# mhw32/multimodal-vae-public

Measured on AMD Instinct MI355X. Metric: images/sec (MVAE train step), higher is better.
Workload: dtype f32; 1 GPU; mnist MVAE train step, n-latents 64, batch 512 per GPU; global_batch=512, parallelism=dp1, launch=hipGraph replay

## Files before the change

### include/mvae_hip.h

```cpp
#ifndef MVAE_HIP_H
#define MVAE_HIP_H

#include <stddef.h>
#include <stdint.h>

#ifdef __cplusplus
extern "C" {
#endif

#define MVAE_OK          0
#define MVAE_ERR_ARG    (-1)
#define MVAE_ERR_LAUNCH (-2)
#define MVAE_ERR_WS     (-3)
#define MVAE_ERR_COMM   (-4)

#define MVAE_ACT_SWISH   1
#define MVAE_ACCUMULATE  2

#define MVAE_POE_VARIANT_A 0
#define MVAE_POE_VARIANT_B 1
#define MVAE_POE_NO_PRIOR  4
#define MVAE_MAX_EXPERTS  32

typedef void *mvae_stream_t;
// ... 137 lines not shown
#define MVAE_LROUTE_G2S_32x32_K4     7
#define MVAE_LROUTE_IGS_64x32_K4     8
#define MVAE_LROUTE_IGS_64x32_K2     9
#define MVAE_LROUTE_IGS_32x64_K4    10
#define MVAE_LROUTE_IGS_32x64_K2    11
#define MVAE_LROUTE_IGS_32x32_K8    12
#define MVAE_LROUTE_IGS_32x32_K4    13
#define MVAE_LROUTE_IG_32x128       14
#define MVAE_LROUTE_IG_128x128      15
#define MVAE_LROUTE_IG_128x64       16
#define MVAE_LROUTE_IG_64x128       17
#define MVAE_LROUTE_IG_64x64_K4     18
#define MVAE_LROUTE_IG_64x64_K2     19
#define MVAE_LROUTE_IG_64x64        20
#define MVAE_LROUTE_IG_32x128_S     30
#define MVAE_LROUTE_IG_128x128_S    31
#define MVAE_LROUTE_IG_128x64_S     32
#define MVAE_LROUTE_IG_64x128_S     33
#define MVAE_LROUTE_IG_64x64_K4_S   34
#define MVAE_LROUTE_IG_64x64_K2_S   35
#define MVAE_LROUTE_IG_64x64_S      36
#define MVAE_LROUTE_DGRAD_SMALLN    40
#define MVAE_LROUTE_WGRAD_DIRECT_4  41
#define MVAE_LROUTE_WGRAD_DIRECT_8  42
#define MVAE_LROUTE_WGRAD_DIRECT_16 43
#define MVAE_LROUTE_WGRAD_BATCHED2      50
#define MVAE_LROUTE_WGRAD_BATCHED       51
#define MVAE_LROUTE_WGRAD_BATCHED_ADAM  52
int mvae_linear_route(int op, int G, int M, int N, int K, int ld_a, int ld_b, size_t gs_a, size_t gs_b, int aligned,
                      int fwd_form, int want_db, size_t ws_bytes, int *splits ,
                      int *finish );
int mvae_linear_wgrad_batched_route(const mvae_wgrad_item *items, int n_items, int adam, int *tile_rows ,
                                    int *tile_cols , int *waves );

int mvae_conv2d_gen_fwd(const float *x, const float *w, float *pre, float *act,
                        int B, int Cin, int H, int W, int Cout, int ks, int stride, int pad,
                        mvae_stream_t stream);
int mvae_conv2d_gen_dgrad(const float *dy, const float *w, float *dx, const float *pre_in,
                          int B, int Cin, int H, int W, int Cout, int ks, int stride, int pad,
                          void *ws, size_t ws_bytes, mvae_stream_t stream);
int mvae_conv2d_gen_wgrad(const float *dy, const float *x, float *dw,
                          int B, int Cin, int H, int W, int Cout, int ks, int stride, int pad,
                          int flags, void *ws, size_t ws_bytes, mvae_stream_t stream);
int mvae_convT2d_gen_fwd(const float *x, const float *w, float *pre, float *act,
                         int B, int Cin, int H, int W, int Cout, int ks, int stride, int pad,
                         void *ws, size_t ws_bytes, mvae_stream_t stream);
int mvae_convT2d_gen_dgrad(const float *dy, const float *w, float *dx, const float *pre_in,
                           int B, int Cin, int H, int W, int Cout, int ks, int stride, int pad,
                           mvae_stream_t stream);
int mvae_convT2d_gen_wgrad(const float *dy, const float *x, float *dw,
                           int B, int Cin, int H, int W, int Cout, int ks, int stride, int pad,
                           int flags, void *ws, size_t ws_bytes, mvae_stream_t stream);
size_t mvae_conv_gen_ws_bytes(int op, int B, int Cin, int H, int W, int Cout, int ks, int stride, int pad);
int mvae_conv_gen_supported(int transposed, int B, int Cin, int H, int W, int Cout, int ks, int stride, int pad);

size_t mvae_bn_ws_bytes(int G, int C, int n_per_group);
int mvae_bn_train_fwd(const float *x, const float *gamma, const float *beta, float *y,
                      float *save_mean, float *save_invstd,
                      float *running_mean, float *running_var,
                      int G, int B, int C, int HW, float eps, float momentum,
                      int n_updates, const int *n_updates_dev ,
                      int flags, void *ws, size_t ws_bytes, mvae_stream_t stream);
int mvae_bn_train_bwd(const float *dy, const float *x, const float *gamma, const float *beta,
                      const float *save_mean, const float *save_invstd,
                      float *dx, float *dgamma, float *dbeta,
                      int G, int B, int C, int HW, int flags,
// ... 325 lines not shown
```

### multimodal-vae-public_amd/_lib.py

```python
import ctypes
import os
from ctypes import c_double, c_float, c_int, c_size_t, c_uint64, c_void_p

_HERE = os.path.dirname(os.path.abspath(__file__))
LIB_PATH = os.path.join(_HERE, 'libmvae_hip.so')

MVAE_OK = 0
ERRORS = {-1: 'MVAE_ERR_ARG (bad shape / null pointer / unsupported stride)',
          -2: 'MVAE_ERR_LAUNCH (hip kernel launch failed)',
          -3: 'MVAE_ERR_WS (workspace too small)',
          -4: 'MVAE_ERR_COMM (RCCL not loadable, or an RCCL / HIP runtime call of mvae_comm_* failed)'}
COMM_ID_BYTES = 128
ACT_SWISH = 1
ACCUMULATE = 2
POE_NO_PRIOR = 4
POE_VARIANT = {'A': 0, 'B': 1, 'A-noprior': 0 | POE_NO_PRIOR, 'B-noprior': 1 | POE_NO_PRIOR}
MAX_EXPERTS = 32
STATS_TILE_ELEMS = 512
MAX_TERMS = 40
CONV_OPS = {'conv_fwd': 0, 'conv_dgrad': 1, 'conv_wgrad': 2, 'convT_fwd': 3, 'convT_fwd_stats': 4, 'convT_dgrad': 5,
            'convT_wgrad': 6}
CONV_ROUTES = {1: 'igemm', 2: 'igemm_pair', 3: 'gemm2', 4: 'conv_patch', 5: 'small_fwd16', 6: 'small_fwd32',
               7: 'dgrad_small3d', 8: 'dgrad_small3', 9: 'dgrad_small2', 10: 'dgrad_small', 11: 's1', 12: 's1_wide',
               13: 'patch8', 14: 'patch7', 15: 'patch16', 16: 'patch_stats', 17: 'wgrad_smallcin',
# ... 105 lines not shown
                                                 c_int, P]),
    'mvae_embedding_swish_bwd_grouped': (c_int, [P, c_int, c_size_t, P, c_size_t, P, c_size_t, P, c_int, c_int,
                                                 c_int, c_int, c_int, P]),
    'mvae_resample_ksize': (c_int, [c_int, c_int]),
    'mvae_resample_coeffs': (c_int, [c_int, c_int, P, P]),
    'mvae_resize_crop_u8_to_f32': (c_int, [P, P] + [c_int] * 8 + [P, P, c_int, P, P, c_int, c_int, c_int, P]),
    'mvae_u8_to_f32': (c_int, [P, P, c_size_t, P]),
    'mvae_poe_fwd': (c_int, [ctypes.POINTER(Experts), c_int, c_int, P, c_int, P, P, P, P, P,
                             c_int, c_int, c_int, P]),
    'mvae_poe_fwd_draw': (c_int, [ctypes.POINTER(Experts), c_int, c_int, P, c_int, P, c_uint64, P, c_uint64, P, P, P, P,
                                  c_int, c_int, c_int, P]),
    'mvae_poe_bwd': (c_int, [ctypes.POINTER(Experts), c_int, c_int, P, c_int, P, P, P, P, P, P, P, c_int,
                             ctypes.POINTER(ExpertGrads), c_int, c_int, c_int, c_int, P]),
    'mvae_poe_bwd_split': (c_int, [ctypes.POINTER(Experts), c_int, c_int, P, c_int, P, P, P, P,
                                   ctypes.POINTER(c_int), P, ctypes.POINTER(c_int), P, c_int,
                                   ctypes.POINTER(ExpertGrads), c_int, c_int, c_int, c_int, P]),
    'mvae_kl_rows_fwd': (c_int, [P, P, P, c_int, c_int, P]),
    'mvae_kl_rows_bwd': (c_int, [P, P, P, P, P, c_int, c_int, P]),
    'mvae_bce_rowsum_fwd': (c_int, [P, P, P, P, P, P] + [c_int] * 7 + [P]),
    'mvae_bce_rowsum_bwd': (c_int, [P, P, P, P, P] + [c_int] * 7 + [P]),
    'mvae_bce_route': (c_int, [c_int] * 4 + [ctypes.POINTER(c_int), ctypes.POINTER(c_int)]),
    'mvae_ce_fwd': (c_int, [P, P, P, P, P, c_int, c_int, c_int, c_int, P]),
    'mvae_ce_bwd': (c_int, [P, P, P, P, c_int, c_int, c_int, c_int, P]),
    'mvae_group_sums': (c_int, [P, P, P, P, c_int, c_int, c_int, P]),
    'mvae_conv_k4_repack_floats': (c_size_t, [c_int, P, c_int, c_int, c_int, c_int, c_int, c_int, c_int]),
    'mvae_conv_k4_repack_batched': (c_int, [ctypes.POINTER(RepackItem), c_int, P]),
    'mvae_convT2d_k4_stats_tiles': (c_size_t, [c_int] * 7),
    'mvae_convT2d_k4_fwd_stats': (c_int, [P, P, P, c_size_t] + [c_int] * 7 + [P, c_size_t, P]),
    'mvae_conv_k4_route': (c_int, [c_int] * 8 + [c_size_t, ctypes.POINTER(c_int)]),
    'mvae_linear_route': (c_int, [c_int] * 7 + [c_size_t, c_size_t, c_int, c_int, c_int, c_size_t, ctypes.POINTER(c_int),
                                  ctypes.POINTER(c_int)]),
    'mvae_linear_wgrad_batched_route': (c_int, [ctypes.POINTER(WgradItem), c_int, c_int, ctypes.POINTER(c_int),
                                                ctypes.POINTER(c_int), ctypes.POINTER(c_int)]),
    'mvae_conv2d_gen_fwd': (c_int, [P, P, P, P] + [c_int] * 8 + [P]),
    'mvae_conv2d_gen_dgrad': (c_int, [P, P, P, P] + [c_int] * 8 + [P, c_size_t, P]),
    'mvae_conv2d_gen_wgrad': (c_int, [P, P, P] + [c_int] * 9 + [P, c_size_t, P]),
    'mvae_convT2d_gen_fwd': (c_int, [P, P, P, P] + [c_int] * 8 + [P, c_size_t, P]),
    'mvae_convT2d_gen_dgrad': (c_int, [P, P, P, P] + [c_int] * 8 + [P]),
    'mvae_convT2d_gen_wgrad': (c_int, [P, P, P] + [c_int] * 9 + [P, c_size_t, P]),
    'mvae_conv_gen_ws_bytes': (c_size_t, [c_int] * 9),
    'mvae_conv_gen_supported': (c_int, [c_int] * 9),
    'mvae_bn_stats_merge': (c_int, [P, c_int, c_int, c_int, c_int, P, P, P, P, c_float, c_float, c_int, P, P]),
    'mvae_linear_wgrad_batched': (c_int, [ctypes.POINTER(WgradItem), c_int, P]),
    'mvae_linear_wgrad_batched_adam': (c_int, [ctypes.POINTER(WgradItem), c_int, ctypes.POINTER(AdamFuse), P]),
    'mvae_adam_prepare': (c_int, [P, ctypes.c_int64, c_double, c_double, c_double, P, P]),
    'mvae_elbo_reduce': (c_int, [ctypes.POINTER(ElboPart), c_int, P, c_int, P, c_size_t, P, c_uint64, P]),
    'mvae_elbo_reduce_prepare': (c_int, [ctypes.POINTER(ElboPart), c_int, P, c_int, P, c_size_t, P, c_uint64, P,
                                         ctypes.c_int64, c_double, c_double, c_double, P, P]),
    'mvae_philox_fill': (c_int, [P, c_size_t, c_int, c_float, c_uint64, P, c_uint64, P]),
    'mvae_randn': (c_int, [P, c_size_t, c_uint64, P, P]),
    'mvae_bernoulli': (c_int, [P, c_size_t, c_float, c_uint64, P, P]),
    'mvae_adam_step': (c_int, [P, P, P, P, c_size_t, c_double, c_double, c_double, c_double, c_float, P, P]),
    'mvae_adam_apply': (c_int, [P, P, P, P, c_size_t, c_double, c_double, c_double, c_double, c_float, P, P]),
    'mvae_adam_apply_at': (c_int, [P, P, P, P, c_size_t, c_double, c_double, c_double, c_double, c_float, P,
                                   ctypes.c_int64, P]),
    'mvae_adam_apply_coef': (c_int, [P, P, P, P, c_size_t, P, c_double, c_double, c_double, c_float, P]),
    'mvae_counter_add': (c_int, [P, ctypes.c_int64, P]),
    'mvae_trace_marker': (c_int, [c_int, P]),
    'mvae_fill': (c_int, [P, c_size_t, c_float, P]),
    'mvae_ingest': (c_int, [P, P, c_size_t, P, P, c_size_t, P, P, c_size_t, P]),
    'mvae_reparam_fwd': (c_int, [P, P, P, P, c_size_t, P]),
    'mvae_reparam_bwd': (c_int, [P, P, P, P, P, c_size_t, P]),
    'mvae_dropout_fanout_fwd': (c_int, [P, P, P, c_float, c_int, c_int, c_int, P]),
    'mvae_dropout_fanin_bwd': (c_int, [P, P, P, c_float, c_int, c_int, c_int, P]),
    'mvae_block_gather': (c_int, [P, P, P, c_int, c_size_t, P]),
    'mvae_block_scatter_add': (c_int, [P, P, P, c_int, c_int, c_size_t, P]),
# ... 94 lines not shown
```

### multimodal-vae-public_amd/csrc/linear.hip

```cpp
#include "gemm_core.h"
#include "gemm2.h"
#include "linear_direct.h"



MVAE_EXPORT int mvae_abi_version(void) { return 6; }

#ifdef MVAE_TUNING
MvaeTune g_mvae_tune = {0, 0, 0, 0, 0, 0, 0, 0};
MVAE_EXPORT void mvae_debug_set_tiling(int wm, int wn, int splits) {
    g_mvae_tune.wm = wm; g_mvae_tune.wn = wn; g_mvae_tune.splits = splits;
}
MVAE_EXPORT void mvae_debug_set_kwaves(int kw) { g_mvae_tune.kw = kw; }
MVAE_EXPORT void mvae_debug_set_small(int off, int waves) { g_mvae_tune.small_off = off; g_mvae_tune.small_waves = waves; }
MVAE_EXPORT void mvae_debug_set_split_target(long blocks) { g_mvae_tune.split_target = blocks; }
MVAE_EXPORT void mvae_debug_set_knockout(int mode) { g_mvae_tune.knockout = mode; }
#endif

MVAE_EXPORT size_t mvae_gemm_ws_bytes(int rows_out, int cols_out, int reduce_len) {
    if (rows_out <= 0 || cols_out <= 0 || reduce_len <= 0) return 0;
    size_t n = split_ws_floats(rows_out, cols_out, reduce_len);
    const size_t repack = (size_t)rows_out * cols_out;
    if (MVAE_TUNE(splits) > 0) n = (size_t)MVAE_TUNE(splits) * ((size_t)rows_out * cols_out + rows_out);
    const size_t smallcin = (size_t)512 * rows_out * cols_out;
// ... 417 lines not shown
        }
        case MVAE_LOP_BCE_FWD: case MVAE_LOP_CE_FWD:
            if (G != 1 || ld_a < K || ld_b < N || (op == MVAE_LOP_CE_FWD && N > 32)) return MVAE_ERR_ARG;
            r = linear_loss_route(a, ld_a, a, M, N, K);
            break;
        case MVAE_LOP_DGRAD:
            if (ld_a < N || ld_b < K) return MVAE_ERR_ARG;
            r = linear_dgrad_route(a, ld_a, a, M, N, K, ws, ws_bytes, gr);
            break;
        case MVAE_LOP_WGRAD:
            if (ld_a < N || ld_b < K) return MVAE_ERR_ARG;
            r = linear_wgrad_route(a, ld_a, a, ld_b, want_db != 0, M, N, K, ws, ws_bytes, gr);
            break;
        default: return MVAE_ERR_ARG;
    }
    if (r.route > 0) {
        if (splits) *splits = r.splits;
        if (finish) *finish = r.finish;
    }
    return r.route;
}

MVAE_EXPORT int mvae_linear_wgrad_batched_route(const mvae_wgrad_item *items, int n_items, int adam, int *tile_rows,
                                                int *tile_cols, int *waves) {
    WgradBatchArgs a;
    const int rc = wgrad_batch_table(items, n_items, adam != 0, a);
    if (rc != MVAE_OK) return rc;
    const WgradBatchRoute r = wgrad_batched_route(a, adam != 0);
    if (tile_rows) *tile_rows = r.tile_m;
    if (tile_cols) *tile_cols = r.tile_n;
    if (waves) *waves = r.waves;
    return r.route;
}
```

### multimodal-vae-public_amd/csrc/linear_direct.h

```cpp
#pragma once
#include "gemm_core.h"

namespace {

#ifdef MVAE_TUNING
#define MVAE_KO1 1
#define MVAE_KO2 2
#else
#define MVAE_KO1 0
#define MVAE_KO2 0
#endif
constexpr int WD_PD = 4;

struct AdamFuse {
    const float *grad_base; float *param, *m, *v; const float *coef;
    float b1, b2, omb1, omb2, eps, gscale;
    __device__ AdamCoef load() const {
        AdamCoef c;
        c.b1 = b1; c.b2 = b2; c.omb1 = omb1; c.omb2 = omb2; c.eps = eps; c.gscale = gscale;
        c.step_size = coef[0]; c.inv_sqrt_bc2 = coef[1];
        return c;
    }
    __device__ void update(const float *gptr, float g, const AdamCoef &c) const {
        const size_t off = (size_t)(gptr - grad_base);
        adam_one(param[off], m[off], v[off], g, c);
    }
};

template <bool ROWSUM, int KW, int MODE = 0, bool ADAM = false>
__device__ __forceinline__ void wgrad_direct_tile(const float *dy, int lddy, const float *x, int ldx,
                                                  const EpRowMajor &e, int I, int J, int M, float *db,
                                                  int db_accumulate, int tile_i, int tile_j,
                                                  const AdamFuse *af = nullptr) {
    extern __shared__ __attribute__((aligned(16))) float wd_lds[];
// ... 157 lines not shown
        for (int el = threadIdx.x; el < ADAM_ONLY_TILE; el += 64 * KW) {
            const int idx = local * ADAM_ONLY_TILE + el;
            if (idx < w.J) af->update(w.dw + idx, w.dw[idx], ac);
        }
        return;
    }
    const int tile_i = local / w.tiles_j, tile_j = local - tile_i * w.tiles_j;
    EpRowMajor e;
    e.out = w.dw; e.act = nullptr; e.ld = w.J; e.bias = nullptr; e.dpre = nullptr; e.ldp = 0;
    e.mask = nullptr; e.ldm = 0; e.mask_scale = 1.f; e.I = w.I; e.J = w.J; e.accumulate = w.accumulate;
    if (w.db) wgrad_direct_tile<true, KW, 0, ADAM>(w.dy, w.lddy, w.x, w.ldx, e, w.I, w.J, w.M, w.db, w.accumulate, tile_i, tile_j, af);
    else wgrad_direct_tile<false, KW, 0, ADAM>(w.dy, w.lddy, w.x, w.ldx, e, w.I, w.J, w.M, nullptr, 0, tile_i, tile_j, af);
}

#ifndef MVAE_WB2_PD22
#define MVAE_WB2_PD22 1
#endif
#ifndef MVAE_WB2_PD11
#define MVAE_WB2_PD11 2
#endif

constexpr int WB2_SEGS = 8;
struct WgradBatch2Args { WgradBatchItem it[WGRAD_BATCH_MAX]; int n; int seg[WB2_SEGS + 1]; };

__device__ __forceinline__ i32x4_t wb2_rsrc(BufBase b, unsigned off, unsigned extent) {
    const unsigned long long a = (((unsigned long long)b.hi << 32) | b.lo) + off;
    i32x4_t r;
    r.x = (int)(unsigned)a; r.y = (int)((unsigned)(a >> 32) & 0xffffu);
    const int left = (int)extent - (int)off;
    r.z = left > 0 ? left : 0; r.w = 0x00020000;
    return r;
}

template <int KW, int FM, int FN, int PD>
__device__ __forceinline__ void wgrad_tile2(const WgradBatchItem &w, int tile_i, int tile_j) {
    extern __shared__ __attribute__((aligned(16))) float wd_lds[];
    constexpr int TM = 32 * FM, TN = 32 * FN;
    const int t = threadIdx.x, lane = t & 63;
    const int kg = __builtin_amdgcn_readfirstlane(t >> 6);
    const int lcol = lane & 31, lrow = lane >> 5;
    const int i0 = tile_i * TM, j0 = tile_j * TN;
    const BufBase ba = buf_base(w.dy), bb = buf_base(w.x);
    const int M = __builtin_amdgcn_readfirstlane(w.M), I = __builtin_amdgcn_readfirstlane(w.I), J = __builtin_amdgcn_readfirstlane(w.J);
    const unsigned ulda = (unsigned)__builtin_amdgcn_readfirstlane(w.lddy) * 4u;
    const unsigned uldb = (unsigned)__builtin_amdgcn_readfirstlane(w.ldx) * 4u;
    const unsigned ext_a = (unsigned)(M - 1) * ulda + (unsigned)I * 4u;
    const unsigned ext_b = (unsigned)(M - 1) * uldb + (unsigned)J * 4u;
    int va[4], vb[4];
#pragma unroll
    for (int q = 0; q < 4; ++q) {
        va[q] = (int)((unsigned)(4 * lrow + q) * ulda + (unsigned)(i0 + lcol) * 4u);
        vb[q] = (int)((unsigned)(4 * lrow + q) * uldb + (unsigned)(j0 + lcol) * 4u);
    }
    const bool rs_block = w.db != nullptr && tile_j == 0;
    f32x16 acc[FM][FN];
#pragma unroll
    for (int a = 0; a < FM; ++a)
#pragma unroll
        for (int b = 0; b < FN; ++b)
#pragma unroll
            for (int r = 0; r < 16; ++r) acc[a][b][r] = 0.f;
    float rs[FM];
#pragma unroll
    for (int a = 0; a < FM; ++a) rs[a] = 0.f;

    const int nchunks = (M + 7) >> 3;
    const int n_it = (nchunks + KW - 1) / KW;
    float a0[PD][FM][4], b0[PD][FN][4], a1[PD][FM][4], b1[PD][FN][4];
    auto load_set = [&](int first, float (&as)[PD][FM][4], float (&bs)[PD][FN][4]) {
#pragma unroll
        for (int p = 0; p < PD; ++p) {
            const unsigned c = (unsigned)(kg + (first + p) * KW);
            const i32x4_t ra = wb2_rsrc(ba, c * 8u * ulda, ext_a), rb = wb2_rsrc(bb, c * 8u * uldb, ext_b);
#pragma unroll
            for (int q = 0; q < 4; ++q) {
#pragma unroll
                for (int f = 0; f < FM; ++f) as[p][f][q] = buf_load1(ra, va[q] + 128 * f);
#pragma unroll
                for (int f = 0; f < FN; ++f) bs[p][f][q] = buf_load1(rb, vb[q] + 128 * f);
            }
        }
    };
    auto use_set = [&](auto with_rs, const float (&as)[PD][FM][4], const float (&bs)[PD][FN][4]) {
#pragma unroll
        for (int p = 0; p < PD; ++p) {
#pragma unroll
            for (int q = 0; q < 4; ++q)
#pragma unroll
                for (int f = 0; f < FM; ++f)
#pragma unroll
                    for (int g = 0; g < FN; ++g)
                        acc[f][g] = __builtin_amdgcn_mfma_f32_32x32x2f32(as[p][f][q], bs[p][g][q], acc[f][g], 0, 0, 0);
            if constexpr (decltype(with_rs)::value) {
#pragma unroll
                for (int f = 0; f < FM; ++f) rs[f] += (as[p][f][0] + as[p][f][1]) + (as[p][f][2] + as[p][f][3]);
            }
        }
    };
    auto main_loop = [&](auto with_rs) {
        load_set(0, a0, b0);
        for (int it = 0; it < n_it; it += 2 * PD) {
            load_set(it + PD, a1, b1);
            __builtin_amdgcn_sched_barrier(0);
            use_set(with_rs, a0, b0);
            __builtin_amdgcn_sched_barrier(0);
            load_set(it + 2 * PD, a0, b0);
            __builtin_amdgcn_sched_barrier(0);
            use_set(with_rs, a1, b1);
            __builtin_amdgcn_sched_barrier(0);
        }
    };
    if (rs_block) main_loop(std::true_type{});
    else main_loop(std::false_type{});
    constexpr int TP = TN + 1;
    constexpr int WTILE = TM * TP;
    auto park = [&](float *dst) {
#pragma unroll
        for (int f = 0; f < FM; ++f)
#pragma unroll
            for (int g = 0; g < FN; ++g)
#pragma unroll
                for (int r = 0; r < 16; ++r)
                    dst[(32 * f + 4 * lrow + (r & 3) + 8 * (r >> 2)) * TP + 32 * g + lcol] = acc[f][g][r];
    };
    float *rsl = wd_lds + (KW > 1 ? KW / 2 : 1) * WTILE;
    if (rs_block) {
#pragma unroll
        for (int f = 0; f < FM; ++f) rsl[(kg * 2 + lrow) * TM + 32 * f + lcol] = rs[f];
    }
#pragma unroll
    for (int half = KW / 2; half >= 1; half >>= 1) {
        if (kg >= half && kg < 2 * half) park(wd_lds + (kg - half) * WTILE);
        __syncthreads();
        if (kg < half) {
            const float *src = wd_lds + kg * WTILE;
#pragma unroll
            for (int f = 0; f < FM; ++f)
#pragma unroll
                for (int g = 0; g < FN; ++g)
#pragma unroll
                    for (int r = 0; r < 16; ++r)
                        acc[f][g][r] += src[(32 * f + 4 * lrow + (r & 3) + 8 * (r >> 2)) * TP + 32 * g + lcol];
        }
        __syncthreads();
    }
    if (kg == 0) park(wd_lds);
    __syncthreads();
    float *dw = w.dw;
    const int acc_flag = w.accumulate;
    constexpr int NE = TM * TN / (64 * KW);
#pragma unroll
    for (int k = 0; k < NE; ++k) {
        const int el = t + k * 64 * KW;
        const int il = el / TN, jl = el % TN;
        const int i = i0 + il, j = j0 + jl;
        if (i < I && j < J) {
            float v = wd_lds[il * TP + jl];
            float *dst = dw + (size_t)i * J + j;
            if (acc_flag) v += *dst;
            *dst = v;
        }
    }
    if (rs_block && t < TM && i0 + t < I) {
        float s2 = 0.f;
#pragma unroll
        for (int g2 = 0; g2 < 2 * KW; ++g2) s2 += rsl[g2 * TM + t];
        if (acc_flag) s2 += w.db[i0 + t];
        w.db[i0 + t] = s2;
    }
}

template <int KW, int FM, int FN, int PD>
__global__ __launch_bounds__(64 * KW) void wgrad_batched2_kernel(WgradBatch2Args a) {
    const int xcd = blockIdx.x & (WB2_SEGS - 1), slot = blockIdx.x >> 3;
    const int tile = a.seg[xcd] + slot;
    if (tile >= a.seg[xcd + 1]) return;
    int p = 0, first = 0;
#pragma unroll 1
    for (int q = 0; q < a.n - 1; ++q) {
        if (tile >= a.it[q].tile_end) { p = q + 1; first = a.it[q].tile_end; }
    }
    const WgradBatchItem &w = a.it[p];
    const int local = tile - first;
    const int tile_i = local / w.tiles_j, tile_j = local - tile_i * w.tiles_j;
    wgrad_tile2<KW, FM, FN, PD>(w, tile_i, tile_j);
}

struct Wgrad2Route { bool ok; int shape, kw; };
inline Wgrad2Route wgrad_batched2_route(const WgradBatchArgs &a) {
    Wgrad2Route none = {false, 0, 0};
    long t22 = 0, t21 = 0, t11 = 0;
    int max_m = 0;
    for (int q = 0; q < a.n; ++q) {
        const WgradBatchItem &w = a.it[q];
        if (!w.dy) return none;
        t22 += cdiv(w.I, 64) * cdiv(w.J, 64); t21 += cdiv(w.I, 64) * cdiv(w.J, 32); t11 += cdiv(w.I, 32) * cdiv(w.J, 32);
        if (w.M > max_m) max_m = w.M;
        const long over = (long)w.M + 8 * 16 * 8;
        if (over * w.lddy * 4 >= (1L << 31) || over * w.ldx * 4 >= (1L << 31)) return none;
    }
    const long busy22 = cdiv(t22, 256) * 4, busy21 = cdiv(t21, 256) * 2, busy11 = cdiv(t11, 256);
    int shape = 22;
    long busy = busy22;
    if (busy21 < busy) { shape = 21; busy = busy21; }
    if (busy11 < busy) { shape = 11; busy = busy11; }
    const long tiles = shape == 22 ? t22 : (shape == 21 ? t21 : t11);
    int kw = tiles >= 1024 ? 2 : (tiles >= 400 ? 4 : (tiles >= 160 ? 8 : 16));
    if (shape == 22 && kw < 4) kw = 4;
    while (kw > 2 && max_m < 8 * 4 * kw) kw >>= 1;
    if (shape == 11 && kw < 4) kw = 4;
    if (kw >= 16) kw = 16;
    else if (kw != 8 && !(kw == 2 && shape == 21)) kw = 4;
    const Wgrad2Route r = {true, shape, kw};
    return r;
}

inline int wgrad_batched2_launch(const WgradBatchArgs &a, const Wgrad2Route &r, hipStream_t st) {
    const int shape = r.shape, kw = r.kw;
    const int fm = shape == 11 ? 1 : 2, fn = shape == 22 ? 2 : 1;
    WgradBatch2Args b;
    b.n = a.n;
    int total = 0;
    for (int q = 0; q < a.n; ++q) {
        b.it[q] = a.it[q];
        b.it[q].tiles_j = (int)cdiv(a.it[q].J, 32 * fn);
        total += (int)cdiv(a.it[q].I, 32 * fm) * b.it[q].tiles_j;
        b.it[q].tile_end = total;
    }
    int longest = 0;
    for (int x = 0; x <= WB2_SEGS; ++x) b.seg[x] = (int)((long)total * x / WB2_SEGS);
    for (int x = 0; x < WB2_SEGS; ++x) if (b.seg[x + 1] - b.seg[x] > longest) longest = b.seg[x + 1] - b.seg[x];
    const dim3 grid((unsigned)(longest * WB2_SEGS));
#define MVAE_WB2(KWV, FMV, FNV, PDV)                                                                          \
    {                                                                                                         \
        constexpr size_t lds = ((size_t)(KWV > 1 ? KWV / 2 : 1) * (32 * FMV) * (32 * FNV + 1) + (size_t)KWV * 2 * 32 * FMV) * sizeof(float); \
        auto kern = wgrad_batched2_kernel<KWV, FMV, FNV, PDV>;                                                \
        static bool attr_done = false;                                                                        \
        if (!attr_done) {                                                                                     \
            (void)hipFuncSetAttribute(reinterpret_cast<const void *>(kern), hipFuncAttributeMaxDynamicSharedMemorySize, (int)lds); \
            attr_done = true;                                                                                 \
        }                                                                                                     \
        hipLaunchKernelGGL(kern, grid, dim3(64 * KWV), lds, st, b);                                           \
    }
    if (shape == 22) {
        if (kw == 16) MVAE_WB2(16, 2, 2, 1) else if (kw == 8) MVAE_WB2(8, 2, 2, MVAE_WB2_PD22) else MVAE_WB2(4, 2, 2, MVAE_WB2_PD22)
    } else if (shape == 21) {
        if (kw == 16) MVAE_WB2(16, 2, 1, 2) else if (kw == 8) MVAE_WB2(8, 2, 1, 2) else if (kw == 4) MVAE_WB2(4, 2, 1, 3) else MVAE_WB2(2, 2, 1, 3)
    } else {
        if (kw == 16) MVAE_WB2(16, 1, 1, MVAE_WB2_PD11) else if (kw == 8) MVAE_WB2(8, 1, 1, MVAE_WB2_PD11) else MVAE_WB2(4, 1, 1, MVAE_WB2_PD11)
    }
#undef MVAE_WB2
    return mvae_launch_status();
}

inline bool wgrad_batch_item_ok(int I, int J, int M, int lddy, int ldx) {
    const long tiles = cdiv(I, 32) * cdiv(J, 32);
    return tiles <= 2048 && M <= 4096 && (long)M * lddy * 4 < (1L << 32) && (long)M * ldx * 4 < (1L << 32);
}

inline int wgrad_batched_waves(int total) { return total >= 768 ? 4 : (total >= 256 ? 8 : 16); }

struct WgradBatchRoute { int route, tile_m, tile_n, waves; Wgrad2Route r2; };
inline WgradBatchRoute wgrad_batched_route(const WgradBatchArgs &a, bool adam) {
    WgradBatchRoute r;
    r.r2.ok = false; r.r2.shape = 0; r.r2.kw = 0;
    if (!adam) r.r2 = wgrad_batched2_route(a);
    if (r.r2.ok) {
        r.route = MVAE_LROUTE_WGRAD_BATCHED2;
        r.tile_m = r.r2.shape == 11 ? 32 : 64; r.tile_n = r.r2.shape == 22 ? 64 : 32; r.waves = r.r2.kw;
    } else {
        r.route = adam ? MVAE_LROUTE_WGRAD_BATCHED_ADAM : MVAE_LROUTE_WGRAD_BATCHED;
        r.tile_m = r.tile_n = 32; r.waves = wgrad_batched_waves(a.it[a.n - 1].tile_end);
    }
    return r;
}

inline int wgrad_batched_launch(WgradBatchArgs &a, hipStream_t st, const AdamFuse *adam = nullptr) {
    const WgradBatchRoute r = wgrad_batched_route(a, adam != nullptr);
    if (r.route == MVAE_LROUTE_WGRAD_BATCHED2) return wgrad_batched2_launch(a, r.r2, st);
    const int total = a.it[a.n - 1].tile_end;
    const int kw = r.waves;
#define MVAE_WB(KWV)                                                                                          \
    {                                                                                                         \
        constexpr size_t lds = ((size_t)KWV * 32 * 33 + (size_t)KWV * 64) * sizeof(float);                    \
        static bool attr_done = false;                                                                        \
// ... 64 lines not shown
```

### multimodal-vae-public_amd/kernels.py

```python
import ctypes

import torch

from . import _lib
from ._lib import ACCUMULATE, ACT_SWISH, check

_WS = {}
_WS_MIN_BYTES = 64 << 20


def _stream():
    return ctypes.c_void_p(torch.cuda.current_stream().cuda_stream)


def _ptr(t):
    return ctypes.c_void_p(t.data_ptr()) if t is not None else None


def _need_gpu(*tensors):
    for t in tensors:
        if t is not None and not t.is_cuda:
            raise RuntimeError('multimodal-vae-public_amd: the HIP path needs GPU tensors (got %s); '
                               'there is no CPU fallback' % t.device)

# ... 104 lines not shown
                if adam is None:
                    raise RuntimeError('update-only items need adam=')
                _need_gpu(dw); _f32c(dw)
                arr[q] = _lib.WgradItem(None, 0, None, 0, _ptr(dw), None, 0, 0, dw.numel(), 0)
                continue
            _need_gpu(dy, x, dw, db); _f32c(dw, db)
            M, N = dy.shape
            if x.shape[0] != M or tuple(dw.shape) != (N, x.shape[1]):
                raise RuntimeError('wgrad item %d: shapes %s %s %s' % (q, tuple(dy.shape), tuple(x.shape), tuple(dw.shape)))
            arr[q] = _lib.WgradItem(_ptr(dy), dy.stride(0), _ptr(x), x.stride(0), _ptr(dw), _ptr(db), M, N,
                                    x.shape[1], ACCUMULATE if acc else 0)
        if adam is not None:
            check(_lib.lib().mvae_linear_wgrad_batched_adam(arr, len(chunk), ctypes.byref(adam), _stream()),
                  'mvae_linear_wgrad_batched_adam')
        else:
            check(_lib.lib().mvae_linear_wgrad_batched(arr, len(chunk), _stream()), 'mvae_linear_wgrad_batched')


def linear_route(op, M, N, K, G=1, ld_a=None, ld_b=None, gs_a=None, gs_b=None, aligned=True, form='other', db=False,
                 ws_bytes=None):
    dense = {'fwd': (K, N, M * K, N * K), 'bce_fwd': (K, N, 0, 0), 'ce_fwd': (K, N, 0, 0),
             'dgrad': (N, K, M * N, N * K), 'wgrad': (N, K, M * N, M * K)}[op]
    ld_a, ld_b, gs_a, gs_b = (d if v is None else v for v, d in zip((ld_a, ld_b, gs_a, gs_b), dense))
    sp, fin = ctypes.c_int(1), ctypes.c_int(0)
    rc = _lib.lib().mvae_linear_route(_lib.LINEAR_OPS[op], G, M, N, K, ld_a, ld_b, gs_a, gs_b, 1 if aligned else 0,
                                      _lib.LINEAR_FORMS[form], 1 if db else 0,
                                      _WS_MIN_BYTES if ws_bytes is None else int(ws_bytes), ctypes.byref(sp),
                                      ctypes.byref(fin))
    if rc <= 0:
        check(rc if rc < 0 else -1, 'mvae_linear_route')
    return _lib.LINEAR_ROUTES[rc], sp.value, _lib.LINEAR_FINISH[fin.value]


def linear_wgrad_batched_route(items, adam=False):
    items = list(items)
    arr = (_lib.WgradItem * max(len(items), 1))()
    for q, it in enumerate(items):
        if len(it) == 7:
            M, N, K, lddy, ldx, with_db, acc = it
            base = (q + 1) << 24
            arr[q] = _lib.WgradItem(base, lddy, base + 16, ldx, base + 32, base + 48 if with_db else None, M, N, K,
                                    ACCUMULATE if acc else 0)
        else:
            dy, x, dw, db, acc = it
            if dy is None:
                arr[q] = _lib.WgradItem(None, 0, None, 0, _ptr(dw), None, 0, 0, dw.numel(), 0)
            else:
                arr[q] = _lib.WgradItem(_ptr(dy), dy.stride(0), _ptr(x), x.stride(0), _ptr(dw), _ptr(db), dy.shape[0],
                                        dy.shape[1], x.shape[1], ACCUMULATE if acc else 0)
    tm, tn, kw = ctypes.c_int(0), ctypes.c_int(0), ctypes.c_int(0)
    rc = _lib.lib().mvae_linear_wgrad_batched_route(arr, len(items), 1 if adam else 0, ctypes.byref(tm), ctypes.byref(tn),
                                                    ctypes.byref(kw))
    if rc <= 0:
        check(rc if rc < 0 else -1, 'mvae_linear_wgrad_batched_route')
    return _lib.LINEAR_ROUTES[rc], (tm.value, tn.value), kw.value


def _g3(t, name):
    if t.dim() != 3 or t.stride(2) != 1 or t.stride(0) < t.shape[1] * t.stride(1):
        raise RuntimeError('%s must be a [groups, rows, width] tensor with unit column stride' % name)
    return t


def linear_fwd_grouped(x, w0, w_gs, b0, b_gs, pre=None, act=None):
    _need_gpu(x, w0, b0, pre, act)
    G, M, K = _g3(x, 'x').shape
    N = w0.shape[0]
    out = _g3(pre if pre is not None else act, 'output')
    if pre is not None and act is not None and (act.stride() != pre.stride()):
        raise RuntimeError('pre and act must share a layout')
    ws, wsb = _ws_args(G * _lib.lib().mvae_gemm_ws_bytes(M, N, K), x.device)
    check(_lib.lib().mvae_linear_fwd_grouped(_ptr(x), x.stride(1), x.stride(0), _ptr(w0), w_gs, _ptr(b0), b_gs,
                                             _ptr(pre), _ptr(act), out.stride(1), out.stride(0), G, M, N, K,
                                             ws, wsb, _stream()), 'mvae_linear_fwd_grouped')


def linear_fwd_grouped_shared(x, G, w0, w_gs, b0, b_gs, pre=None, act=None):
    _need_gpu(x, w0, b0, pre, act)
    M, K = _rows2d(x, 'x').shape
    N = w0.shape[0]
    out = _g3(pre if pre is not None else act, 'output')
    if out.shape[0] != int(G) or out.shape[1] != M or out.shape[2] != N:
        raise RuntimeError('output must be [%d, %d, %d], got %s' % (G, M, N, tuple(out.shape)))
    if pre is not None and act is not None and (act.stride() != pre.stride()):
        raise RuntimeError('pre and act must share a layout')
    ws, wsb = _ws_args(int(G) * _lib.lib().mvae_gemm_ws_bytes(M, N, K), x.device)
    check(_lib.lib().mvae_linear_fwd_grouped(_ptr(x), x.stride(0), 0, _ptr(w0), w_gs, _ptr(b0), b_gs, _ptr(pre), _ptr(act),
                                             out.stride(1), out.stride(0), int(G), M, N, K, ws, wsb, _stream()),
# ... 1290 lines not shown
```

Baseline: 2.001 million images/sec.

## Stream wgrad batched2 operands through an LDS ring with direct-to-LDS loads

Adds a ring-buffered path to the batched weight-gradient kernel. Global loads of dy and x go straight into a multi-stage LDS ring using direct-to-LDS loads, with 16-byte pieces when alignment allows and 4-byte pieces otherwise, and explicit vmcnt/lgkmcnt waits overlap the loads with the MFMA work. It also sets a waves-per-EU occupancy hint, makes the ring path the default, and adds a query API plus a tuning env switch to turn it off. The larger LDS footprint and the hand-written waitcnt scheduling can lower occupancy or introduce hazards if the counts are wrong.

```diff
diff --git a/include/mvae_hip.h b/include/mvae_hip.h
--- a/include/mvae_hip.h
+++ b/include/mvae_hip.h
@@ -193,6 +193,9 @@
                       int *finish );
 int mvae_linear_wgrad_batched_route(const mvae_wgrad_item *items, int n_items, int adam, int *tile_rows ,
                                     int *tile_cols , int *waves );
+int mvae_linear_wgrad_ring_query(const mvae_wgrad_item *items, int n_items, int *piece_dy ,
+                                 int *piece_x , int *depth ,
+                                 int *lds_bytes );
 
 int mvae_conv2d_gen_fwd(const float *x, const float *w, float *pre, float *act,
                         int B, int Cin, int H, int W, int Cout, int ks, int stride, int pad,
diff --git a/multimodal-vae-public_amd/_lib.py b/multimodal-vae-public_amd/_lib.py
--- a/multimodal-vae-public_amd/_lib.py
+++ b/multimodal-vae-public_amd/_lib.py
@@ -161,6 +161,8 @@
                                   ctypes.POINTER(c_int)]),
     'mvae_linear_wgrad_batched_route': (c_int, [ctypes.POINTER(WgradItem), c_int, c_int, ctypes.POINTER(c_int),
                                                 ctypes.POINTER(c_int), ctypes.POINTER(c_int)]),
+    'mvae_linear_wgrad_ring_query': (c_int, [ctypes.POINTER(WgradItem), c_int, ctypes.POINTER(c_int),
+                                             ctypes.POINTER(c_int), ctypes.POINTER(c_int), ctypes.POINTER(c_int)]),
     'mvae_conv2d_gen_fwd': (c_int, [P, P, P, P] + [c_int] * 8 + [P]),
     'mvae_conv2d_gen_dgrad': (c_int, [P, P, P, P] + [c_int] * 8 + [P, c_size_t, P]),
     'mvae_conv2d_gen_wgrad': (c_int, [P, P, P] + [c_int] * 9 + [P, c_size_t, P]),
diff --git a/multimodal-vae-public_amd/csrc/linear.hip b/multimodal-vae-public_amd/csrc/linear.hip
--- a/multimodal-vae-public_amd/csrc/linear.hip
+++ b/multimodal-vae-public_amd/csrc/linear.hip
@@ -473,3 +473,21 @@
     if (waves) *waves = r.waves;
     return r.route;
 }
+
+MVAE_EXPORT int mvae_linear_wgrad_ring_query(const mvae_wgrad_item *items, int n_items, int *piece_dy, int *piece_x,
+                                             int *depth, int *lds_bytes) {
+    WgradBatchArgs a;
+    const int rc = wgrad_batch_table(items, n_items, false, a);
+    if (rc != MVAE_OK) return rc;
+    const WgradBatchRoute r = wgrad_batched_route(a, false);
+    const bool ring = r.route == MVAE_LROUTE_WGRAD_BATCHED2;
+    const Wgrad2RingInfo info = ring ? wgrad_batched2_ring(r.r2) : Wgrad2RingInfo{0, 0};
+    for (int q = 0; q < n_items; ++q) {
+        const WgradBatchItem &w = a.it[q];
+        if (piece_dy) piece_dy[q] = !ring ? 0 : (wb2_piece16((unsigned long long)(uintptr_t)w.dy, w.lddy, w.I) ? 16 : 4);
+        if (piece_x) piece_x[q] = !ring ? 0 : (wb2_piece16((unsigned long long)(uintptr_t)w.x, w.ldx, w.J) ? 16 : 4);
+    }
+    if (depth) *depth = info.depth;
+    if (lds_bytes) *lds_bytes = info.lds_bytes;
+    return r.route;
+}
diff --git a/multimodal-vae-public_amd/csrc/linear_direct.h b/multimodal-vae-public_amd/csrc/linear_direct.h
--- a/multimodal-vae-public_amd/csrc/linear_direct.h
+++ b/multimodal-vae-public_amd/csrc/linear_direct.h
@@ -1,5 +1,5 @@
 #pragma once
-#include "gemm_core.h"
+#include "gemm2.h"
 
 namespace {
 
@@ -223,7 +223,24 @@
     return r;
 }
 
-template <int KW, int FM, int FN, int PD>
+template <int KW, int FM, int FN> struct Wb2Ring {
+    static constexpr int A_FLOATS = 8 * 32 * FM, CH = 8 * 32 * (FM + FN);
+    static constexpr int CAP = 96 * 1024;
+    static constexpr int FIT = CAP / (KW * CH * 4);
+    static constexpr int S = FIT >= 4 ? 4 : (FIT >= 2 ? FIT : 2);
+    static constexpr size_t RING_BYTES = (size_t)KW * S * CH * sizeof(float);
+    static constexpr size_t RED_BYTES = ((size_t)(KW > 1 ? KW / 2 : 1) * (32 * FM) * (32 * FN + 1) + (size_t)KW * 2 * 32 * FM) * sizeof(float);
+    static constexpr size_t LDS_BYTES = RING_BYTES > RED_BYTES ? RING_BYTES : RED_BYTES;
+};
+__host__ __device__ inline bool wb2_piece16(unsigned long long p, int ld, int width) {
+    return (p & 15ull) == 0 && (ld & 3) == 0 && (width & 3) == 0;
+}
+template <int N> __device__ __forceinline__ void wb2_wait_vm() {
+    static_assert(N >= 0 && N <= 63, "vmcnt is 6 bits");
+    asm volatile("s_waitcnt vmcnt(%0)" ::"n"(N) : "memory");
+}
+
+template <int KW, int FM, int FN, int PD, bool RING>
 __device__ __forceinline__ void wgrad_tile2(const WgradBatchItem &w, int tile_i, int tile_j) {
     extern __shared__ __attribute__((aligned(16))) float wd_lds[];
     constexpr int TM = 32 * FM, TN = 32 * FN;
@@ -237,26 +254,125 @@
     const unsigned uldb = (unsigned)__builtin_amdgcn_readfirstlane(w.ldx) * 4u;
     const unsigned ext_a = (unsigned)(M - 1) * ulda + (unsigned)I * 4u;
     const unsigned ext_b = (unsigned)(M - 1) * uldb + (unsigned)J * 4u;
+    const bool rs_block = w.db != nullptr && tile_j == 0;
+    f32x16 acc[FM][FN];
+#pragma unroll
+    for (int a = 0; a < FM; ++a)
+#pragma unroll
+        for (int b = 0; b < FN; ++b)
+#pragma unroll
+            for (int r = 0; r < 16; ++r) acc[a][b][r] = 0.f;
+    float rs[FM];
+#pragma unroll
+    for (int a = 0; a < FM; ++a) rs[a] = 0.f;
+
+    const int nchunks = (M + 7) >> 3;
+    const int n_it = (nchunks + KW - 1) / KW;
+    if constexpr (RING) {
+        using R = Wb2Ring<KW, FM, FN>;
+        constexpr int S = R::S, CH = R::CH, AF = R::A_FLOATS;
+        const unsigned ring0 = (unsigned)(unsigned long)(g2_lds_void *)wd_lds + (unsigned)(kg * S * CH * 4);
+        const bool a16 = __builtin_amdgcn_readfirstlane((int)wb2_piece16(ba.lo, (int)(ulda >> 2), I)) != 0;
+        const bool b16 = __builtin_amdgcn_readfirstlane((int)wb2_piece16(bb.lo, (int)(uldb >> 2), J)) != 0;
+        const int c4 = lane & 7, h16 = (lane >> 3) & 1;
+        const int q16a = FM == 2 ? lane >> 5 : lane >> 4, f16a = FM == 2 ? (lane >> 4) & 1 : 0;
+        const int q16b = FN == 2 ? lane >> 5 : lane >> 4, f16b = FN == 2 ? (lane >> 4) & 1 : 0;
+        const int voa = a16 ? (int)((unsigned)(4 * h16 + q16a) * ulda + (unsigned)(i0 + 32 * f16a + 4 * c4) * 4u)
+                            : (int)((unsigned)(4 * lrow) * ulda + (unsigned)(i0 + lcol) * 4u);
+        const int vob = b16 ? (int)((unsigned)(4 * h16 + q16b) * uldb + (unsigned)(j0 + 32 * f16b + 4 * c4) * 4u)
+                            : (int)((unsigned)(4 * lrow) * uldb + (unsigned)(j0 + lcol) * 4u);
+        auto issue = [&](auto A16, auto B16, int it, int st) {
+            const unsigned c = (unsigned)(kg + it * KW);
+            const unsigned dst = ring0 + (unsigned)(st * CH * 4);
+            if constexpr (decltype(A16)::value) {
+#pragma unroll
+                for (int u = 0; u < FM; ++u)
+                    g2_dma16(wb2_rsrc(ba, (c * 8u + (FM == 2 ? 2u * u : 0u)) * ulda, ext_a), voa, dst + 1024u * u);
+            } else {
+#pragma unroll
+                for (int q = 0; q < 4; ++q)
+#pragma unroll
+                    for (int f = 0; f < FM; ++f)
+                        g2_dma4(wb2_rsrc(ba, (c * 8u + q) * ulda + 128u * f, ext_a), voa, 0, dst + 256u * (q * FM + f));
+            }
+            if constexpr (decltype(B16)::value) {
+#pragma unroll
+                for (int u = 0; u < FN; ++u)
+                    g2_dma16(wb2_rsrc(bb, (c * 8u + (FN == 2 ? 2u * u : 0u)) * uldb, ext_b), vob, dst + 4u * AF + 1024u * u);
+            } else {
+#pragma unroll
+                for (int q = 0; q < 4; ++q)
+#pragma unroll
+                    for (int f = 0; f < FN; ++f)
+                        g2_dma4(wb2_rsrc(bb, (c * 8u + q) * uldb + 128u * f, ext_b), vob, 0, dst + 4u * AF + 256u * (q * FN + f));
+            }
+        };
+        auto landed = [&](auto A16, auto B16) {
+            wb2_wait_vm<(S - 1) * ((decltype(A16)::value ? FM : 4 * FM) + (decltype(B16)::value ? FN : 4 * FN))>();
+        };
+        auto fetch = [&](int st, float (&as)[FM][4], float (&bs)[FN][4]) {
+            const float *p = wd_lds + (kg * S + st) * CH + lane;
+#pragma unroll
+            for (int q = 0; q < 4; ++q) {
+#pragma unroll
+                for (int f = 0; f < FM; ++f) as[f][q] = p[(q * FM + f) * 64];
+#pragma unroll
+                for (int f = 0; f < FN; ++f) bs[f][q] = p[AF + (q * FN + f) * 64];
+            }
+        };
+        auto mfmas = [&](int q, const float (&as)[FM][4], const float (&bs)[FN][4]) {
+#pragma unroll
+            for (int f = 0; f < FM; ++f)
+#pragma unroll
+                for (int g = 0; g < FN; ++g)
+                    acc[f][g] = __builtin_amdgcn_mfma_f32_32x32x2f32(as[f][q], bs[g][q], acc[f][g], 0, 0, 0);
+        };
+        float a0[FM][4], b0[FN][4], a1[FM][4], b1[FN][4];
+        int st = 0;
+        auto step = [&](auto with_rs, auto A16, auto B16, int it, const float (&as)[FM][4], const float (&bs)[FN][4], float (&an)[FM][4], float (&bn)[FN][4]) {
+            landed(A16, B16);
+            st = st + 1 == S ? 0 : st + 1;
+            fetch(st, an, bn);
+            __builtin_amdgcn_sched_barrier(0);
+            mfmas(0, as, bs); mfmas(1, as, bs);
+            __builtin_amdgcn_sched_barrier(0);
+            asm volatile("s_waitcnt lgkmcnt(0)" ::: "memory");
+            issue(A16, B16, it + 1 + S, st);
+            __builtin_amdgcn_sched_barrier(0);
+            mfmas(2, as, bs); mfmas(3, as, bs);
+            if constexpr (decltype(with_rs)::value) {
+#pragma unroll
+                for (int f = 0; f < FM; ++f) rs[f] += (as[f][0] + as[f][1]) + (as[f][2] + as[f][3]);
+            }
+            __builtin_amdgcn_sched_barrier(0);
+        };
+        auto main_loop = [&](auto with_rs, auto A16, auto B16) {
+#pragma unroll
+            for (int s = 0; s < S; ++s) issue(A16, B16, s, s);
+            landed(A16, B16);
+            fetch(0, a0, b0);
+            asm volatile("s_waitcnt lgkmcnt(0)" ::: "memory");
+            issue(A16, B16, S, 0);
+            for (int it = 0; it < n_it; it += 2) {
+                step(with_rs, A16, B16, it, a0, b0, a1, b1);
+                step(with_rs, A16, B16, it + 1, a1, b1, a0, b0);
+            }
+        };
+        auto by_pieces = [&](auto with_rs) {
+            if (a16) { if (b16) main_loop(with_rs, std::true_type{}, std::true_type{}); else main_loop(with_rs, std::true_type{}, std::false_type{}); }
+            else { if (b16) main_loop(with_rs, std::false_type{}, std::true_type{}); else main_loop(with_rs, std::false_type{}, std::false_type{}); }
+        };
+        if (rs_block) by_pieces(std::true_type{});
+        else by_pieces(std::false_type{});
+        asm volatile("s_waitcnt vmcnt(0)" ::: "memory");
+        __syncthreads();
+    } else {
     int va[4], vb[4];
 #pragma unroll
     for (int q = 0; q < 4; ++q) {
         va[q] = (int)((unsigned)(4 * lrow + q) * ulda + (unsigned)(i0 + lcol) * 4u);
         vb[q] = (int)((unsigned)(4 * lrow + q) * uldb + (unsigned)(j0 + lcol) * 4u);
     }
-    const bool rs_block = w.db != nullptr && tile_j == 0;
-    f32x16 acc[FM][FN];
-#pragma unroll
-    for (int a = 0; a < FM; ++a)
-#pragma unroll
-        for (int b = 0; b < FN; ++b)
-#pragma unroll
-            for (int r = 0; r < 16; ++r) acc[a][b][r] = 0.f;
-    float rs[FM];
-#pragma unroll
-    for (int a = 0; a < FM; ++a) rs[a] = 0.f;
-
-    const int nchunks = (M + 7) >> 3;
-    const int n_it = (nchunks + KW - 1) / KW;
     float a0[PD][FM][4], b0[PD][FN][4], a1[PD][FM][4], b1[PD][FN][4];
     auto load_set = [&](int first, float (&as)[PD][FM][4], float (&bs)[PD][FN][4]) {
 #pragma unroll
@@ -303,6 +419,7 @@
     };
     if (rs_block) main_loop(std::true_type{});
     else main_loop(std::false_type{});
+    }
     constexpr int TP = TN + 1;
     constexpr int WTILE = TM * TP;
     auto park = [&](float *dst) {
@@ -361,8 +478,10 @@
     }
 }
 
-template <int KW, int FM, int FN, int PD>
-__global__ __launch_bounds__(64 * KW) void wgrad_batched2_kernel(WgradBatch2Args a) {
+constexpr int wb2_waves(int kw, int fm, int fn) { return fm * fn == 1 ? 8 : (kw >= 8 ? 4 : 3); }
+template <int KW, int FM, int FN, int PD, bool RING>
+__global__ __launch_bounds__(64 * KW) __attribute__((amdgpu_waves_per_eu(wb2_waves(KW, FM, FN))))
+void wgrad_batched2_kernel(WgradBatch2Args a) {
     const int xcd = blockIdx.x & (WB2_SEGS - 1), slot = blockIdx.x >> 3;
     const int tile = a.seg[xcd] + slot;
     if (tile >= a.seg[xcd + 1]) return;
@@ -374,7 +493,7 @@
     const WgradBatchItem &w = a.it[p];
     const int local = tile - first;
     const int tile_i = local / w.tiles_j, tile_j = local - tile_i * w.tiles_j;
-    wgrad_tile2<KW, FM, FN, PD>(w, tile_i, tile_j);
+    wgrad_tile2<KW, FM, FN, PD, RING>(w, tile_i, tile_j);
 }
 
 struct Wgrad2Route { bool ok; int shape, kw; };
@@ -422,10 +541,15 @@
     for (int x = 0; x <= WB2_SEGS; ++x) b.seg[x] = (int)((long)total * x / WB2_SEGS);
     for (int x = 0; x < WB2_SEGS; ++x) if (b.seg[x + 1] - b.seg[x] > longest) longest = b.seg[x + 1] - b.seg[x];
     const dim3 grid((unsigned)(longest * WB2_SEGS));
-#define MVAE_WB2(KWV, FMV, FNV, PDV)                                                                          \
+#ifdef MVAE_TUNING
+    static const bool ring_off = getenv("MVAE_WB2_RING_OFF") != nullptr;
+#else
+    constexpr bool ring_off = false;
+#endif
+#define MVAE_WB2_GO(KWV, FMV, FNV, PDV, RINGV, LDSV)                                                          \
     {                                                                                                         \
-        constexpr size_t lds = ((size_t)(KWV > 1 ? KWV / 2 : 1) * (32 * FMV) * (32 * FNV + 1) + (size_t)KWV * 2 * 32 * FMV) * sizeof(float); \
-        auto kern = wgrad_batched2_kernel<KWV, FMV, FNV, PDV>;                                                \
+        constexpr size_t lds = LDSV;                                                                          \
+        auto kern = wgrad_batched2_kernel<KWV, FMV, FNV, PDV, RINGV>;                                         \
         static bool attr_done = false;                                                                        \
         if (!attr_done) {                                                                                     \
             (void)hipFuncSetAttribute(reinterpret_cast<const void *>(kern), hipFuncAttributeMaxDynamicSharedMemorySize, (int)lds); \
@@ -433,6 +557,16 @@
         }                                                                                                     \
         hipLaunchKernelGGL(kern, grid, dim3(64 * KWV), lds, st, b);                                           \
     }
+#ifdef MVAE_TUNING
+#define MVAE_WB2(KWV, FMV, FNV, PDV)                                                                          \
+    {                                                                                                         \
+        if (ring_off) MVAE_WB2_GO(KWV, FMV, FNV, PDV, false, (Wb2Ring<KWV, FMV, FNV>::RED_BYTES))             \
+        else MVAE_WB2_GO(KWV, FMV, FNV, PDV, true, (Wb2Ring<KWV, FMV, FNV>::LDS_BYTES))                       \
+    }
+#else
+#define MVAE_WB2(KWV, FMV, FNV, PDV) MVAE_WB2_GO(KWV, FMV, FNV, PDV, true, (Wb2Ring<KWV, FMV, FNV>::LDS_BYTES))
+#endif
+    (void)ring_off;
     if (shape == 22) {
         if (kw == 16) MVAE_WB2(16, 2, 2, 1) else if (kw == 8) MVAE_WB2(8, 2, 2, MVAE_WB2_PD22) else MVAE_WB2(4, 2, 2, MVAE_WB2_PD22)
     } else if (shape == 21) {
@@ -441,7 +575,18 @@
         if (kw == 16) MVAE_WB2(16, 1, 1, MVAE_WB2_PD11) else if (kw == 8) MVAE_WB2(8, 1, 1, MVAE_WB2_PD11) else MVAE_WB2(4, 1, 1, MVAE_WB2_PD11)
     }
 #undef MVAE_WB2
+#undef MVAE_WB2_GO
     return mvae_launch_status();
+}
+
+struct Wgrad2RingInfo { int depth, lds_bytes; };
+inline Wgrad2RingInfo wgrad_batched2_ring(const Wgrad2Route &r) {
+#define MVAE_WB2_INFO(KWV, FMV, FNV) Wgrad2RingInfo{Wb2Ring<KWV, FMV, FNV>::S, (int)Wb2Ring<KWV, FMV, FNV>::LDS_BYTES}
+    const int kw = r.kw;
+    if (r.shape == 22) return kw == 16 ? MVAE_WB2_INFO(16, 2, 2) : (kw == 8 ? MVAE_WB2_INFO(8, 2, 2) : MVAE_WB2_INFO(4, 2, 2));
+    if (r.shape == 21) return kw == 16 ? MVAE_WB2_INFO(16, 2, 1) : (kw == 8 ? MVAE_WB2_INFO(8, 2, 1) : (kw == 4 ? MVAE_WB2_INFO(4, 2, 1) : MVAE_WB2_INFO(2, 2, 1)));
+    return kw == 16 ? MVAE_WB2_INFO(16, 1, 1) : (kw == 8 ? MVAE_WB2_INFO(8, 1, 1) : MVAE_WB2_INFO(4, 1, 1));
+#undef MVAE_WB2_INFO
 }
 
 inline bool wgrad_batch_item_ok(int I, int J, int M, int lddy, int ldx) {
diff --git a/multimodal-vae-public_amd/kernels.py b/multimodal-vae-public_amd/kernels.py
--- a/multimodal-vae-public_amd/kernels.py
+++ b/multimodal-vae-public_amd/kernels.py
@@ -160,15 +160,16 @@
     return _lib.LINEAR_ROUTES[rc], sp.value, _lib.LINEAR_FINISH[fin.value]
 
 
-def linear_wgrad_batched_route(items, adam=False):
+def _route_items(items):
     items = list(items)
     arr = (_lib.WgradItem * max(len(items), 1))()
     for q, it in enumerate(items):
-        if len(it) == 7:
-            M, N, K, lddy, ldx, with_db, acc = it
+        if len(it) in (7, 9):
+            M, N, K, lddy, ldx, with_db, acc = it[:7]
+            ody, ox = it[7:] if len(it) == 9 else (0, 0)
             base = (q + 1) << 24
-            arr[q] = _lib.WgradItem(base, lddy, base + 16, ldx, base + 32, base + 48 if with_db else None, M, N, K,
-                                    ACCUMULATE if acc else 0)
+            arr[q] = _lib.WgradItem(base + ody, lddy, base + 16 + ox, ldx, base + 32, base + 48 if with_db else None,
+                                    M, N, K, ACCUMULATE if acc else 0)
         else:
             dy, x, dw, db, acc = it
             if dy is None:
@@ -176,12 +177,27 @@
             else:
                 arr[q] = _lib.WgradItem(_ptr(dy), dy.stride(0), _ptr(x), x.stride(0), _ptr(dw), _ptr(db), dy.shape[0],
                                         dy.shape[1], x.shape[1], ACCUMULATE if acc else 0)
+    return arr, len(items)
+
+
+def linear_wgrad_batched_route(items, adam=False):
+    arr, n = _route_items(items)
     tm, tn, kw = ctypes.c_int(0), ctypes.c_int(0), ctypes.c_int(0)
-    rc = _lib.lib().mvae_linear_wgrad_batched_route(arr, len(items), 1 if adam else 0, ctypes.byref(tm), ctypes.byref(tn),
+    rc = _lib.lib().mvae_linear_wgrad_batched_route(arr, n, 1 if adam else 0, ctypes.byref(tm), ctypes.byref(tn),
                                                     ctypes.byref(kw))
     if rc <= 0:
         check(rc if rc < 0 else -1, 'mvae_linear_wgrad_batched_route')
     return _lib.LINEAR_ROUTES[rc], (tm.value, tn.value), kw.value
+
+
+def linear_wgrad_ring(items):
+    arr, n = _route_items(items)
+    pa, px = (ctypes.c_int * max(n, 1))(), (ctypes.c_int * max(n, 1))()
+    depth, lds = ctypes.c_int(0), ctypes.c_int(0)
+    rc = _lib.lib().mvae_linear_wgrad_ring_query(arr, n, pa, px, ctypes.byref(depth), ctypes.byref(lds))
+    if rc <= 0:
+        check(rc if rc < 0 else -1, 'mvae_linear_wgrad_ring_query')
+    return _lib.LINEAR_ROUTES[rc], [(pa[q], px[q]) for q in range(n)], depth.value, lds.value
 
 
 def _g3(t, name):
```

Result: no change. 2.019 million images/sec (median of 6 runs) (+0.9%).
